# NeLy-EPFL/DeepFly3D

Measured on AMD Instinct MI355X. Metric: frames/sec (7-view 2D->3D), higher is better.
Workload: dtype f32; 1 GPU; BASELINE configs[1]: 2176 frames x 7 views 256x512x3 per GPU, 2-stack hourglass fp32, arg-max + 38-joint layout + fp64 DLT; frames_per_gpu=2176, parallelism=frame-sharded x1, one packed gather, collective_executed=False

## Files before the change

### deepfly3d_amd/csrc/hg_bt_common.h

```cpp
#pragma once
#include "hg_bt_reg.h"
#include "hg_types.h"

namespace hgk {

constexpr int BR_STAGE_BYTES = 8192;
constexpr int BR_RING = 4;
constexpr int BR_RING_BYTES = BR_RING * BR_STAGE_BYTES;
constexpr int BR_T1_PITCH = 128 * 2;
constexpr int BR_T1_BYTES = BT_HALO * BR_T1_PITCH;
__device__ __forceinline__ int br_t1_swz(int hp) { return (hp % BT_HW) & 15; }
__host__ __device__ constexpr int br_swz(int r, int c) { return (r >> 2) * 256 + (((((r & 3) << 2) | c) ^ ((r >> 3) & 3)) << 4); }
__device__ __forceinline__ void br_barrier() { asm volatile("s_waitcnt lgkmcnt(0)\n\ts_barrier" ::: "memory"); }

__device__ __forceinline__ float br_relu(float x) {
    const int b = __builtin_bit_cast(int, x);
    return __builtin_bit_cast(float, b > 0 ? b : 0);
}

template <typename I>
__device__ __forceinline__ int bt_xcd_block(I id, int n) {
    const int xcd = id & 7, q = n >> 3, r = n & 7;
    return (xcd < r ? xcd * (q + 1) : r * (q + 1) + (xcd - r) * q) + (id >> 3);
}
struct BtTile { int tx0, ty0, view; };
template <int TW, int TH, typename I>
__device__ __forceinline__ BtTile bt_tile(I id, int n, int tiles_x, int tiles_y) {
    const int b = bt_xcd_block(id, n), tx0 = (b % tiles_x) * TW, by = b / tiles_x;
    return BtTile{tx0, (by % tiles_y) * TH, by / tiles_y};
}

__device__ __forceinline__ void br_ring_issue(const void* stream, int stage, unsigned slot_addr, int wave, unsigned wvoff) {
    br_glds_stage(reinterpret_cast<const unsigned char*>(stream) + (size_t)stage * BR_STAGE_BYTES, wvoff, slot_addr + (unsigned)wave * 2048);
}

template <int HW, int HALO, int ROWB>
__device__ __forceinline__ void bt_t1_issue(const unsigned char* tin, const void* zeros, const int& tx0, const int& ty0, const int& H, const int& W, int koff,
                                            unsigned t1_addr, const int& wave, const int& lane) {
#ifdef BRF_NO_T1DMA
    return;
#endif
#pragma unroll
    for (int k = 0; k < (HALO / 4 + 3) / 4; ++k) {
        const int pc = wave + 4 * k;
        if (pc < HALO / 4) {
            const int hp = 4 * pc + (lane >> 4);
            const int hy = hp / HW, hx = hp % HW;
            const int y = ty0 - 1 + hy, x = tx0 - 1 + hx;
            const bool ok = (unsigned)y < (unsigned)H && (unsigned)x < (unsigned)W;
            const unsigned chunk = (unsigned)((lane & 15) ^ ((hp % HW) & 15));
            const unsigned char* const src = ok ? tin + ((size_t)y * W + x) * ROWB + koff + chunk * 16 : reinterpret_cast<const unsigned char*>(zeros) + chunk * 16;
            br_glds_piece64(src, t1_addr + (unsigned)pc * 1024u);
        }
    }
}
template <int HW, int HALO, int ROWB, int NH>
__device__ __forceinline__ void bt_t1_issue_persistent(const void* t1in, const void* zeros, int view, int tx0, int ty0, int H, int W, unsigned t1_addr,
                                                       int wave, unsigned uoff) {
    static_assert(NH == 1 || NH == 2, "one 64-channel half, or both");
    int lane_ = (int)(uoff >> 4);
    asm volatile("" : "+v"(lane_));
    int wave_ = wave;
    asm volatile("" : "+s"(wave_));
    const unsigned char* const tin = reinterpret_cast<const unsigned char*>(t1in) + (size_t)view * H * W * ROWB;
    const unsigned char* const zer = reinterpret_cast<const unsigned char*>(zeros);
    const int q = lane_ >> 4, slot = lane_ & 15;
    static_assert(HW >= 16, "one wrap per step of 16 halo pixels");
    const int hp0 = 4 * wave_ + q;
    int hy = hp0 / HW, hx = hp0 - hy * HW;
#pragma unroll
    for (int k = 0; k < (HALO / 4 + 3) / 4; ++k) {
        const int pc = wave_ + 4 * k;
        if (pc < HALO / 4) {
            const int y = ty0 - 1 + hy, x = tx0 - 1 + hx;
            const bool ok = (unsigned)y < (unsigned)H && (unsigned)x < (unsigned)W;
            const unsigned c16 = (unsigned)((slot ^ (hx & 15)) << 4);
            const unsigned in_view = (unsigned)((y * W + x) * ROWB) + c16;
            const unsigned char* const src = (ok ? tin : zer) + (ok ? in_view : c16);
            br_glds_piece64(src, t1_addr + (unsigned)(pc * 1024));
            if constexpr (NH == 2) br_glds_piece64(src + (ok ? 256u : 0u), t1_addr + (unsigned)(HALO * 256 + pc * 1024));
        }
        hx += 16;
        if (hx >= HW) {
            hx -= HW;
            ++hy;
        }
    }
}

template <int NT>
__device__ __forceinline__ void bt_t2_start(const float* b2, int half, f32x16 (&t2)[NT]) {
#pragma unroll
    for (int m = 0; m < NT; ++m)
#pragma unroll
        for (int q = 0; q < 4; ++q) {
            const f32x4 bb = *reinterpret_cast<const f32x4*>(b2 + 32 * m + 8 * q + 4 * half);
#pragma unroll
            for (int e = 0; e < 4; ++e) t2[m][4 * q + e] = bb[e];
        }
}
}
```

### deepfly3d_amd/csrc/hg_bt_wino_f32.h

```cpp
#pragma once
#include "hg_bt_common.h"
#include "hg_bt_reg.h"
#include "hg_bt_ring_f32.h"
#include "hg_types.h"

#ifndef WN_ABL
#define WN_ABL 0
#endif

namespace hgk {

constexpr int WN_CHUNKS = 16;
constexpr int WN_PASSES = 6;
#ifndef WN_UBUF
#define WN_UBUF 3
#endif
constexpr int WN_PASS_BYTES = 4 * 4 * 1024;
constexpr int WN_U_BYTES = 64 * WN_PASS_BYTES;
constexpr int WN_U2_BYTES = (WN_CHUNKS * WN_PASSES - 64) * WN_PASS_BYTES;
constexpr int WN_W3_BYTES = BRF_W3_STAGES * BR_STAGE_BYTES;
constexpr int WN_STREAM_BYTES = WN_U_BYTES + WN_W3_BYTES;
constexpr int WN_STREAM_BYTES_L2 = WN_U_BYTES + 2 * WN_W3_BYTES;
constexpr int WN_V_BYTES = 12 * 1024;
constexpr int WN_T1_OFF = BR_RING_BYTES;
constexpr int WN_T1_BYTES = 2 * BR_T1_BYTES;
constexpr int WN_T2_BYTES = BT_TH * BT_TW * 512;
constexpr int WN_B3_OFF = WN_T1_OFF + WN_T1_BYTES;
constexpr int WN_RING2_OFF = WN_B3_OFF + 1024 + 512;
constexpr int WN_LDS_BYTES = WN_RING2_OFF + BR_RING_BYTES;
static_assert(WN_LDS_BYTES <= 160 * 1024, "one workgroup per CU");
static_assert(WN_PASSES % WN_UBUF == 0 && WN_UBUF >= 2, "a chunk's passes use the same buffers in every chunk");
static_assert(WN_V_BYTES <= BR_RING_BYTES / 2, "V buffers 0, 1 in the W3 ring's slots 0 .. 3, buffer 2 in slots 4 .. 7");
static_assert(WN_T2_BYTES <= WN_T1_BYTES, "t2 lives in the t1 region");
static_assert(WN_U2_BYTES <= BRF_NSTAGE * BR_STAGE_BYTES, "U's second part fits the direct-form stage images");

__host__ __device__ constexpr int wn_row(int pg, int q4) { return pg >= 3 ? 3 - (q4 & 1) : (q4 & 1); }
__host__ __device__ constexpr int wn_col(int pg, int q4) { return 2 * (pg % 3) + (q4 >> 1); }

__global__ __launch_bounds__(256) void bt_wino_pack_kernel(const float* __restrict__ w2, float* __restrict__ ustream, float* __restrict__ ustream2) {
    const int idx = blockIdx.x * 256 + threadIdx.x;
    if (idx >= 128 * 128) return;
    const int co = idx >> 7, ci = idx & 127;
    double g[3][3];
#pragma unroll
    for (int ky = 0; ky < 3; ++ky)
#pragma unroll
        for (int kx = 0; kx < 3; ++kx) g[ky][kx] = (double)w2[((size_t)(ky * 3 + kx) * 128 + co) * 128 + ci];
    double t[4][3];
#pragma unroll
    for (int kx = 0; kx < 3; ++kx) {
        t[0][kx] = g[0][kx];
        t[1][kx] = 0.5 * (g[0][kx] + g[1][kx] + g[2][kx]);
        t[2][kx] = 0.5 * (g[0][kx] - g[1][kx] + g[2][kx]);
        t[3][kx] = g[2][kx];
    }
    const int c = ci >> 3, s = (ci >> 2) & 1, k = ci & 3, w = co >> 5, m = (co >> 4) & 1, r = co & 15;
#pragma unroll
    for (int pg = 0; pg < 6; ++pg)
#pragma unroll
        for (int q4 = 0; q4 < 4; ++q4) {
            const double* const x = t[wn_row(pg, q4)];
            double u;
            switch (wn_col(pg, q4)) {
                case 0: u = x[0]; break;
                case 1: u = (x[0] + x[1] + x[2]) / 3.0; break;
                case 2: u = (-x[0] + x[1] - x[2]) / 3.0; break;
                case 3: u = -(16.0 * x[0] + 8.0 * x[1] + 4.0 * x[2]) / 15.0; break;
                case 4: u = (x[0] - 2.0 * x[1] + 4.0 * x[2]) / 15.0; break;
                default: u = x[2]; break;
            }
            const int P = 6 * c + 3 * s + (pg >> 1);
            const size_t off = ((size_t)((P & 63) * 4 + w) * 4 + (pg & 1) * 2 + m) * 256 + (r + 16 * k) * 4 + q4;
            (P < 64 ? ustream : ustream2)[off] = (float)u;
        }
}
__global__ __launch_bounds__(256) void bt_wino_pack_w3_kernel(const float* __restrict__ w3, unsigned char* __restrict__ stream) {
    const int idx = blockIdx.x * 256 + threadIdx.x;
    if (idx >= BRF_W3_STAGES * 512) return;
    const int k = idx >> 9, rem = idx & 511, c = rem & 3, r = rem >> 2, nh = k >> 3, k8 = k & 7;
    const int ch = 4 * (r & 31) + (r >> 5);
    *reinterpret_cast<u32x4*>(stream + (size_t)k * BR_STAGE_BYTES + br_swz(r, c)) = *reinterpret_cast<const u32x4*>(w3 + ((size_t)nh * 128 + ch) * 128 + 16 * k8 + 4 * c);
}

__device__ __forceinline__ void wn_uload4(f32x4 (&d)[4], const void* sbase, unsigned voff) {
    asm volatile("s_nop 4\n\tglobal_load_dwordx4 %0, %4, %5\n\tglobal_load_dwordx4 %1, %4, %5 offset:1024\n\t"
                 "global_load_dwordx4 %2, %4, %5 offset:2048\n\tglobal_load_dwordx4 %3, %4, %5 offset:3072"
                 : "=&v"(d[0]), "=&v"(d[1]), "=&v"(d[2]), "=&v"(d[3])
                 : "v"(voff), "s"(sbase)
                 : "memory");
}
template <int N>
__device__ __forceinline__ void wn_uwait(f32x4 (&u)[4]) {
    asm volatile("s_waitcnt vmcnt(%4)" : "+v"(u[0]), "+v"(u[1]), "+v"(u[2]), "+v"(u[3]) : "n"(N) : "memory");
}
__device__ __forceinline__ unsigned wn_far_off(unsigned off) {
    asm volatile("" : "+s"(off));
    return off;
}
__device__ __forceinline__ void wn_xload1(f32x4& d, const void* sbase, unsigned voff) {
    asm volatile("s_nop 4\n\tglobal_load_dwordx4 %0, %1, %2" : "=&v"(d) : "v"(voff), "s"(sbase) : "memory");
}
template <int STEP>
__device__ __forceinline__ void wn_xload4s(f32x4 (&d)[4], const void* sbase, unsigned voff) {
    asm volatile("s_nop 4\n\tglobal_load_dwordx4 %0, %4, %5\n\tglobal_load_dwordx4 %1, %4, %5 offset:%6\n\t"
                 "global_load_dwordx4 %2, %4, %5 offset:%7\n\tglobal_load_dwordx4 %3, %4, %5 offset:%8"
                 : "=&v"(d[0]), "=&v"(d[1]), "=&v"(d[2]), "=&v"(d[3])
                 : "v"(voff), "s"(sbase), "n"(STEP), "n"(2 * STEP), "n"(3 * STEP)
                 : "memory");
}

template <bool UP, bool ADD2 = false, bool L2 = false>
__global__ __launch_bounds__(256, 1) void bottleneck_wino_f32_kernel(BtRingArgs p) {
    static_assert(!(UP && ADD2), "the fused up-path sum is written by plain blocks");
    static_assert(!L2 || (!UP && !ADD2), "layer2 is a plain block");
    using T = float;
    constexpr int CIN = L2 ? 128 : 256, CO = 256;
    extern __shared__ __attribute__((aligned(16))) unsigned char smem[];
    unsigned char* const ring = smem;
    unsigned char* const t1_lds = smem + WN_T1_OFF;
    float* const b3_lds = reinterpret_cast<float*>(smem + WN_B3_OFF);
    float* const b2_lds = b3_lds + 256;
    const unsigned ring_addr = lds_addr(ring), t1_addr = lds_addr(t1_lds);

    const int tid = threadIdx.x, lane = tid & 63;
    const int wave = __builtin_amdgcn_readfirstlane(tid >> 6);
    const int tiles_x = p.W / BT_TW, tiles_y = p.H / BT_TH;
    const int ntiles = p.V * tiles_y * tiles_x;
    auto tile_of = [&](int vb, int& tx0, int& ty0, int& view) {
        const BtTile t = bt_tile<BT_TW, BT_TH>(vb, ntiles, tiles_x, tiles_y);
        tx0 = t.tx0, ty0 = t.ty0, view = t.view;
    };
    unsigned uoff = (unsigned)(lane * 16);
    asm volatile("" : "+v"(uoff));
    auto t1_issue = [&](int tx0, int ty0, int view) {
        bt_t1_issue_persistent<BT_HW, BT_HALO, 512, 2>(p.t1in, p.zeros, view, tx0, ty0, p.H, p.W, t1_addr, wave, uoff);
    };


    const unsigned char* const ubase = reinterpret_cast<const unsigned char*>(p.w2d) + (size_t)wave * 4096;
    const unsigned char* const ubase2 = reinterpret_cast<const unsigned char*>(p.wstream) + (size_t)wave * 4096 - (size_t)64 * WN_PASS_BYTES;
    auto uload = [&](int c, int e, f32x4 (&dst)[4]) {
        const int P = WN_PASSES * c + e;
        wn_uload4(dst, (P < 64 ? ubase : ubase2) + (size_t)P * WN_PASS_BYTES, uoff);
    };

    const int wh = wave & 1;
    unsigned rd[6], vwr, vrd;
    auto lane_consts = [&]() {
        int l = (int)(uoff >> 4);
        asm volatile("" : "+v"(l));
        const int ppc = l & 3, pte = (l >> 2) & 3, pkq = (l >> 4) & 1, ppr = 2 * (wave >> 1) + (l >> 5);
#pragma unroll
        for (int col = 0; col < 6; ++col) {
            const int hx = 4 * ppc + col, hp = (2 * ppr + wh) * BT_HW + hx;
            rd[col] = (unsigned)(hp * 256 + ((pkq ^ (hx & 15)) << 4) + 4 * pte);
        }
        vwr = (unsigned)(((pkq * 6 + 3 * wh) * 4 + pte) * 256 + (((4 * ppr + ppc) ^ (4 * pte)) << 4));
        vrd = (unsigned)((l >> 4) * 256 + (((l & 15) ^ (4 * (l >> 4))) << 4));
    };
    auto vbuf_off = [](int b) { return b == 0 ? 0 : b == 1 ? BR_RING_BYTES / 2 : WN_RING2_OFF; };
    unsigned vrd2 = 0, vwr2 = 0;
    auto vrd_of = [&](int b) { return b == 2 ? smem + vrd2 : smem + vbuf_off(b) + vrd; };
    const f32x2 cw2 = {-1.0f, wh ? 0.0f : 1.0f}, cw0 = {0.0f, wh ? -1.0f : 0.0f};
    float tR[6][3];
    unsigned ta[6];
    auto t_addr = [&](int c) {
#pragma unroll
        for (int col = 0; col < 6; ++col) {
            ta[col] = (rd[col] ^ (unsigned)((c & 7) << 5)) + (t1_addr + (unsigned)((c >> 3) * BR_T1_BYTES));
            asm volatile("" : "+v"(ta[col]));
        }
    };
    auto t_read = [&](int col) {
        typedef const __attribute__((address_space(3))) float* lds_f;
        if (WN_ABL & 512) {
            asm volatile("" : "+v"(tR[col][0]), "+v"(tR[col][1]), "+v"(tR[col][2]));
            return;
        }
#pragma unroll
        for (int t = 0; t < 3; ++t) tR[col][t] = *(lds_f)(size_t)(ta[col] + t * BT_HW * 256);
    };
    f32x4 vo[3];
    auto t_transform = [&](int c_next_addr) {
        f32x2 x[6];
#pragma unroll
        for (int col = 0; col < 6; ++col) {
            const f32x2 P = {tR[col][0], tR[col][1]};
            if (WN_ABL & 2048) {
                x[col] = P;
                continue;
            }
            x[col] = cw0 * f32x2{tR[col][0], tR[col][0]} + (cw2 * f32x2{tR[col][2], tR[col][2]} + P);
        }
        f32x2 v[6];
        if (WN_ABL & 2048) {
#pragma unroll
            for (int j = 0; j < 6; ++j) v[j] = x[j];
        } else {
            const f32x2 h = {0.5f, 0.5f}, two = {2.0f, 2.0f};
            const f32x2 d13 = x[3] - x[1], d24 = x[4] - x[2];
            v[0] = h * d13 + (((x[0] + x[4]) - two * x[2]) + d13);
            v[1] = h * x[3] + (two * x[3] + (h * x[2] + (x[4] - x[1])));
            v[2] = h * x[3] + (((x[4] + x[1]) - two * x[2]) - h * x[2]);
            v[3] = two * (x[3] - x[1]) + d24;
            v[4] = h * (x[1] - x[3]) + d24;
            v[5] = h * d24 + (((x[5] + x[1]) - two * x[3]) + d24);
        }
#pragma unroll
        for (int jp = 0; jp < 3; ++jp) vo[jp] = f32x4{v[2 * jp][0], v[2 * jp][1], v[2 * jp + 1][0], v[2 * jp + 1][1]};
        t_addr(c_next_addr);
    };
    auto v_store = [&](int buf, int jp) {
        if (WN_ABL & 1024) {
            asm volatile("" ::"v"(vo[jp]));
            return;
        }
        *reinterpret_cast<f32x4*>((buf == 2 ? smem + vwr2 : smem + vbuf_off(buf) + vwr) + jp * 1024) = vo[jp];
    };
    auto t_transform_write = [&](int buf, int c_next_addr) {
        t_transform(c_next_addr);
#pragma unroll
        for (int jp = 0; jp < 3; ++jp) v_store(buf, jp);
    };
    auto ring_slot = [](int k) { return (k & 7) < 4 ? (k & 7) * BR_STAGE_BYTES : WN_RING2_OFF + ((k & 7) - 4) * BR_STAGE_BYTES; };
    auto ring_issue8 = [&](int set) {
        unsigned wvoff = (unsigned)wave * 2048u + uoff;
        asm volatile("" : "+v"(wvoff));
#pragma unroll
        for (int k = 8 * set; k < 8 * set + 8; ++k)
            br_ring_issue(reinterpret_cast<const unsigned char*>(p.w2d) + WN_U_BYTES, k, ring_addr + (unsigned)ring_slot(k), wave, wvoff);
    };

#ifdef DF3D_BT_TIMING
    unsigned long long stamp_ = __builtin_amdgcn_s_memtime();
#endif
    int vb = blockIdx.x;
    int tx0, ty0, view;
    tile_of(vb, tx0, ty0, view);
    t1_issue(tx0, ty0, view);
    b3_lds[tid] = L2 ? p.b3[tid] + p.bd[tid] : p.b3[tid];
    if (tid < 128) b2_lds[tid] = p.b2[tid];
    bool first = true;

#pragma unroll 1
    for (;;) {
        const int vbn = vb + (int)gridDim.x;
        const bool has_next = vbn < ntiles;
        int ntx0 = 0, nty0 = 0, nview = 0;
        if (has_next) tile_of(vbn, ntx0, nty0, nview);
        const size_t ftile = (((size_t)view * p.H + ty0 + 2 * wave) * p.W + tx0) * (CO * 4);
        const size_t htile = (((size_t)view * (p.H / 2) + ty0 / 2 + wave) * (p.W / 2) + tx0 / 2) * (CO * 4);
        const unsigned char* const xtile = reinterpret_cast<const unsigned char*>(p.in) + (L2 ? ftile / 2 : ftile);

        f32x4 acc[48];
        f32x4 ufr[WN_UBUF][4];
#pragma unroll
        for (int e = 0; e < WN_UBUF - 1; ++e) uload(0, e, ufr[e]);
        if (first) asm volatile("s_waitcnt vmcnt(%0)" ::"n"(4 * (WN_UBUF - 1)) : "memory");
        first = false;
        br_barrier();
        BR_STAMP(0);
        lane_consts();
        t_addr(0);
#pragma unroll
        for (int col = 0; col < 6; ++col) t_read(col);
        t_transform_write(0, 1);
#pragma unroll
        for (int col = 0; col < 6; ++col) t_read(col);
        t_transform_write(1, 2);
        br_barrier();
        BR_STAMP(1);

        f32x4 vf[2][2];
        auto chunk = [&](int c, auto br_tag, auto first_tag) {
            constexpr int BR = decltype(br_tag)::value;
            constexpr bool FIRST = decltype(first_tag)::value;
            const int cn = c + 1 < WN_CHUNKS ? c + 1 : c;
            const int c3 = c + 3 < WN_CHUNKS ? c + 3 : WN_CHUNKS - 1;
            const unsigned char* const vb_ = vrd_of(BR);
            if (FIRST) {
#pragma unroll
                for (int g = 0; g < 2; ++g) vf[0][g] = *reinterpret_cast<const f32x4*>(vb_ + g * 1024);
            }
#pragma unroll
            for (int e = 0; e < WN_PASSES; ++e) {
                const int pp = e % 3;
                __builtin_amdgcn_sched_barrier(0);
                if (!(WN_ABL & 1)) {
                    wn_uwait<4 * (WN_UBUF - 2)>(ufr[e % WN_UBUF]);
                    const int eu = e + WN_UBUF - 1;
                    if (eu < WN_PASSES) uload(c, eu, ufr[eu % WN_UBUF]);
                    else uload(cn, eu - WN_PASSES, ufr[eu % WN_UBUF]);
                    __builtin_amdgcn_sched_barrier(0);
                }
                if (e == 3) {
                    if (BR == 0) {
                        vwr2 = vwr + wn_far_off(WN_RING2_OFF);
                        asm volatile("" : "+v"(vwr2));
                    }
                    if (BR == 1) {
                        vrd2 = vrd + wn_far_off(WN_RING2_OFF);
                        asm volatile("" : "+v"(vrd2));
                    }
                    if (!(WN_ABL & 2)) {
                        if (WN_ABL & 4096) t_transform_write((BR + 2) % 3, c3);
                        else t_transform(c3);
                    }
                    __builtin_amdgcn_sched_barrier(0);
                }
#pragma unroll
                for (int g = 0; g < 4; ++g) {
                    if (g < 2) {
                        const int en = e + 1, sn = en / 3, ppn = en % 3;
                        if (e < WN_PASSES - 1) vf[en & 1][g] = *reinterpret_cast<const f32x4*>(vb_ + (sn * 6 + 2 * ppn + g) * 1024);
                        else vf[0][g] = *reinterpret_cast<const f32x4*>(vrd_of((BR + 1) % 3) + g * 1024);
                    }
                    if (e < 2 && g < 3 && !(WN_ABL & 2)) t_read(3 * e + g);
                    if (e == 3 && g < 3 && !(WN_ABL & (2 | 4096))) v_store((BR + 2) % 3, g);
                    const int pgl = g >> 1, m = g & 1, ai = ((2 * pp + pgl) * 2 + m) * 4;
#pragma unroll
                    for (int q4 = 0; q4 < 4; ++q4) {
                        if (FIRST && e < 3)
                            acc[ai + q4] = __builtin_amdgcn_mfma_f32_16x16x4f32(ufr[e % WN_UBUF][2 * pgl + m][q4], vf[e & 1][pgl][q4], f32x4{0.0f, 0.0f, 0.0f, 0.0f}, 0, 0, 0);
                        else
                            acc[ai + q4] = __builtin_amdgcn_mfma_f32_16x16x4f32(ufr[e % WN_UBUF][2 * pgl + m][q4], vf[e & 1][pgl][q4], acc[ai + q4], 0, 0, 0);
                    }
                    __builtin_amdgcn_sched_barrier(0);
                }
            }
            if (!(WN_ABL & 4)) br_barrier();
        };
        chunk(0, std::integral_constant<int, 0>{}, std::true_type{});
#pragma unroll 1
        for (int c = 1; c < WN_CHUNKS; c += 3) {
            chunk(c, std::integral_constant<int, 1>{}, std::false_type{});
            chunk(c + 1, std::integral_constant<int, 2>{}, std::false_type{});
            chunk(c + 2, std::integral_constant<int, 0>{}, std::false_type{});
        }
        if (!(WN_ABL & 1)) {
#pragma unroll
            for (int e = 0; e < WN_UBUF - 1; ++e) wn_uwait<0>(ufr[e]);
        }

        BR_STAMP(2);
        int lane3 = (int)(uoff >> 4);
        asm volatile("" : "+v"(lane3));
        const int half3 = lane3 >> 5, l31_3 = lane3 & 31;
        const unsigned char* const wf0 = ring + br_swz(l31_3, half3);
        const unsigned char* const wf1 = ring + br_swz(l31_3, 2 + half3);
        const int py = 2 * wave + (l31_3 >> 4), px = l31_3 & 15;
        const unsigned lane_full = (unsigned)((4 * half3 * CO + 4 * l31_3) * 4);
        const unsigned lane_half = (unsigned)((2 * half3 * CO + 4 * l31_3) * 4);
        ring_issue8(0);

        if (WN_ABL & 16) {
            float keep = 0.0f;
#pragma unroll
            for (int k = 0; k < 48; ++k) keep += acc[k][0];
            *reinterpret_cast<float*>(t1_lds + lane3 * 4) = keep;
        } else {
            const int q3 = lane3 >> 4, opr = (lane3 & 15) >> 2, opc = lane3 & 3;
#pragma unroll
            for (int m = 0; m < 2; ++m) {
                f32x4 y[2][4];
                const f32x4 bb = *reinterpret_cast<const f32x4*>(b2_lds + 32 * wave + 16 * m + 4 * q3);
#pragma unroll
                for (int reg = 0; reg < 4; ++reg) {
                    float M[4][6];
#pragma unroll
                    for (int pg = 0; pg < 6; ++pg)
#pragma unroll
                        for (int q4 = 0; q4 < 4; ++q4) M[wn_row(pg, q4)][wn_col(pg, q4)] = acc[(pg * 2 + m) * 4 + q4][reg];
                    M[1][1] += bb[reg];
                    float s[2][6];
#pragma unroll
                    for (int j = 0; j < 6; ++j) {
                        s[0][j] = M[0][j] + M[1][j] + M[2][j];
                        s[1][j] = M[1][j] - M[2][j] - M[3][j];
                    }
#pragma unroll
                    for (int a = 0; a < 2; ++a) {
                        const float sa = s[a][1] + s[a][2], sb = s[a][1] - s[a][2];
                        y[a][0][reg] = br_relu(s[a][0] + sa + s[a][3] + s[a][4]);
                        y[a][1][reg] = br_relu(sb + 0.5f * s[a][3] - 2.0f * s[a][4]);
                        y[a][2][reg] = br_relu(sa + 0.25f * s[a][3] + 4.0f * s[a][4]);
                        y[a][3][reg] = br_relu(sb + 0.125f * s[a][3] - 8.0f * s[a][4] + s[a][5]);
                    }
                }
                const int ch = 8 * wave + 4 * m + q3;
#pragma unroll
                for (int a = 0; a < 2; ++a)
#pragma unroll
                    for (int b = 0; b < 4; ++b) {
                        const int yy = 2 * opr + a, xx = 4 * opc + b;
                        *reinterpret_cast<f32x4*>(t1_lds + (yy * BT_TW + xx) * 512 + (((ch ^ (xx & 15) ^ (opr & 1)) & 31) << 4)) = y[a][b];
                    }
            }
        }
        BR_STAMP(3);
        br_wait_vm(0);
        br_barrier();
        f32x16 t2[4];
        {
            const unsigned rbase = (unsigned)((py * BT_TW + px) * 512 + ((half3 ^ (px & 15) ^ (wave & 1)) << 4));
#pragma unroll
            for (int m = 0; m < 4; ++m)
#pragma unroll
                for (int g = 0; g < 4; ++g) {
                    const f32x4 v = *reinterpret_cast<const f32x4*>(t1_lds + (rbase ^ (unsigned)((8 * m + 2 * g) << 4)));
#pragma unroll
                    for (int e = 0; e < 4; ++e) t2[m][4 * g + e] = v[e];
                }
        }

        br_barrier();
        if (has_next && !(WN_ABL & 32)) t1_issue(ntx0, nty0, nview);
        f32x4 xres[1][16];
        f32x4 exv[4];
        static_assert(!(UP && ADD2), "one extra operand");
        auto res_issue = [&](int nh) {
#pragma unroll
            for (int g = 0; g < 4; ++g) {
                if (WN_ABL & 64) {
#pragma unroll
                    for (int j = 0; j < 4; ++j) xres[0][4 * g + j] = f32x4{0.0f, 0.0f, 0.0f, 0.0f};
                } else {
                    wn_uload4(*reinterpret_cast<f32x4(*)[4]>(&xres[0][4 * g]), xtile + ((size_t)(g >> 1) * p.W + 8 * (g & 1)) * (CIN * 4) + nh * 512, lane_full);
                }
            }
            if constexpr (ADD2 || UP) {
#pragma unroll
                for (int key = 0; key < 4; ++key)
                    wn_xload1(exv[key], reinterpret_cast<const unsigned char*>(ADD2 ? p.add2 : p.in2) + htile + ((key & 1) + 4 * (key >> 1)) * (CO * 4) + nh * 512, lane_half);
            }
        };
        auto res_wait = [&](auto n_tag) {
            constexpr int N = decltype(n_tag)::value;
#pragma unroll
            for (int g = 0; g < 4; ++g) wn_uwait<N>(*reinterpret_cast<f32x4(*)[4]>(&xres[0][4 * g]));
            if constexpr (ADD2 || UP) wn_uwait<N>(exv);
        };
        if constexpr (L2) {
#pragma unroll
            for (int r = 0; r < 16; ++r)
                xres[0][r] = *reinterpret_cast<const f32x4*>(xtile + (8 * r) * 4 + (unsigned)((((l31_3 >> 4) * p.W + (l31_3 & 15)) * CIN + 4 * half3) * 4));
        } else {
            res_issue(0);
        }
        BR_STAMP(4);
#pragma unroll
        for (int nh = 0; nh < 2; ++nh) {
            f32x16 o[4];
            if (nh == 1) {
                br_wait_vm(L2 ? 16 : (ADD2 || UP) ? 36 : 32);
                br_barrier();
            }
#pragma unroll
            for (int i = 0; i < 4; ++i) {
                const float bias = b3_lds[nh * 128 + 4 * l31_3 + i];
#pragma unroll
                for (int r = 0; r < 16; ++r) o[i][r] = bias;
            }
            auto kloop = [&](auto skip_tag) {
                constexpr bool SKIP = decltype(skip_tag)::value;
#pragma unroll
                for (int k8 = 0; k8 < 8; ++k8) {
                    const int tile = k8 >> 1, q2 = k8 & 1;
#pragma unroll
                    for (int jj = 0; jj < 2; ++jj)
#pragma unroll
                        for (int i = 0; i < 4; ++i) {
                            const f32x4 wf = *reinterpret_cast<const f32x4*>((jj ? wf1 : wf0) + ring_slot(k8) + i * 2048);
                            if (WN_ABL & 256) {
                                o[i][0] += wf[0];
                                continue;
                            }
                            if constexpr (SKIP) {
                                const f32x4 xa = xres[0][2 * k8 + jj];
                                mfma_quad<T>(xa[0], xa[1], xa[2], xa[3], wf, o[i]);
                            } else {
                                mfma_quad<T>(t2[tile][8 * q2 + 4 * jj], t2[tile][8 * q2 + 4 * jj + 1], t2[tile][8 * q2 + 4 * jj + 2], t2[tile][8 * q2 + 4 * jj + 3], wf, o[i]);
                            }
                        }
                }
            };
            kloop(std::false_type{});
            if constexpr (L2) {
                br_barrier();
                ring_issue8(2 + nh);
                br_wait_vm(0);
                br_barrier();
                kloop(std::true_type{});
            }
            if (nh == 0) {
                br_barrier();
                ring_issue8(1);
            }
            BR_STAMP(5 + 2 * nh);
            if constexpr (!L2) {
                if (!(WN_ABL & 64)) {
                    if (nh == 0) res_wait(std::integral_constant<int, 16>{});
                    else res_wait(std::integral_constant<int, 0>{});
                }
            }
#pragma unroll
            for (int key = 0; key < 4; ++key) {
                const int r0 = 2 * (key & 1) + 4 * (key >> 1);
                const int hoff = ((key & 1) + 4 * (key >> 1)) * (CO * 4) + nh * 512;
                f32x4 xv[4], ov[4];
#pragma unroll
                for (int t = 0; t < 4; ++t) xv[t] = L2 ? f32x4{0.0f, 0.0f, 0.0f, 0.0f} : xres[0][r0 + (t & 1) + 8 * (t >> 1)];
                if constexpr (UP) {
#pragma unroll
                    for (int t = 0; t < 4; ++t) xv[t] += exv[key];
                }
#pragma unroll
                for (int t = 0; t < 4; ++t) {
                    const int r = r0 + (t & 1) + 8 * (t >> 1);
                    ov[t] = f32x4{o[0][r], o[1][r], o[2][r], o[3][r]};
                    if constexpr (!L2) ov[t] += xv[t];
                    if constexpr (ADD2) ov[t] += exv[key];
                    const int pl0 = (r & 3) + 8 * (r >> 2);
                    if (!(WN_ABL & 128) || ov[t][0] == 12345.678f)
                        *reinterpret_cast<f32x4*>(reinterpret_cast<unsigned char*>(p.out) + ftile + ((size_t)(pl0 >> 4) * p.W + (pl0 & 15)) * (CO * 4) + nh * 512 + lane_full) = ov[t];
                }
                auto max4 = [](const f32x4 (&v)[4]) {
                    f32x4 m;
#pragma unroll
                    for (int e = 0; e < 4; ++e) m[e] = fmaxf(fmaxf(v[0][e], v[1][e]), fmaxf(v[2][e], v[3][e]));
                    return m;
                };
                if constexpr (!UP && !L2) if (p.pool_in)
                    *reinterpret_cast<f32x4*>(reinterpret_cast<unsigned char*>(p.pool_in) + htile + hoff + lane_half) = max4(xv);
                if (p.pool) *reinterpret_cast<f32x4*>(reinterpret_cast<unsigned char*>(p.pool) + htile + hoff + lane_half) = max4(ov);
            }
            BR_STAMP(6 + 2 * nh);
            if constexpr (!L2) {
                if (nh == 0) res_issue(1);
            }
        }
        if (!has_next) break;
        vb = vbn;
        tx0 = ntx0;
        ty0 = nty0;
        view = nview;
    }
}

}
```

Before: 754.2 frames/s.

## Defer next-tile halo prefetch into the epilogue k-loop to overlap with MFMA

Moves the DMA issue of the next tile's t1 halo out of its single spot after the barrier. By default it is spread piecewise across the second-half epilogue k-loop, interleaved with the MFMA steps, and the vmcnt waits are adjusted to account for the outstanding halo loads. The aim is to stop the halo loads competing with the residual loads at the start of the epilogue and to hide their latency behind compute. In exchange the vmcnt accounting becomes more intricate, and there is a new wait before the next tile's U loads to drain the epilogue stores.

After: 756.8 frames/s, median of 6. About the same (+0.3%).

```diff
diff --git a/deepfly3d_amd/csrc/hg_bt_common.h b/deepfly3d_amd/csrc/hg_bt_common.h
--- a/deepfly3d_amd/csrc/hg_bt_common.h
+++ b/deepfly3d_amd/csrc/hg_bt_common.h
@@ -88,6 +88,27 @@
     }
 }
 
+template <int HW, int HALO, int ROWB, int NH>
+__device__ __forceinline__ void bt_t1_issue_piece(const void* t1in, const void* zeros, int view, int tx0, int ty0, int H, int W, unsigned t1_addr,
+                                                  int wave, unsigned uoff, int k) {
+    static_assert(NH == 1 || NH == 2, "one 64-channel half, or both");
+    int lane_ = (int)(uoff >> 4);
+    asm volatile("" : "+v"(lane_));
+    const int pc = wave + 4 * k;
+    if (pc >= HALO / 4) return;
+    const unsigned char* const tin = reinterpret_cast<const unsigned char*>(t1in) + (size_t)view * H * W * ROWB;
+    const unsigned char* const zer = reinterpret_cast<const unsigned char*>(zeros);
+    const int hp = 4 * pc + (lane_ >> 4), slot = lane_ & 15;
+    const int hy = hp / HW, hx = hp - hy * HW;
+    const int y = ty0 - 1 + hy, x = tx0 - 1 + hx;
+    const bool ok = (unsigned)y < (unsigned)H && (unsigned)x < (unsigned)W;
+    const unsigned c16 = (unsigned)((slot ^ (hx & 15)) << 4);
+    const unsigned in_view = (unsigned)((y * W + x) * ROWB) + c16;
+    const unsigned char* const src = (ok ? tin : zer) + (ok ? in_view : c16);
+    br_glds_piece64(src, t1_addr + (unsigned)(pc * 1024));
+    if constexpr (NH == 2) br_glds_piece64(src + (ok ? 256u : 0u), t1_addr + (unsigned)(HALO * 256 + pc * 1024));
+}
+
 template <int NT>
 __device__ __forceinline__ void bt_t2_start(const float* b2, int half, f32x16 (&t2)[NT]) {
 #pragma unroll
diff --git a/deepfly3d_amd/csrc/hg_bt_wino_f32.h b/deepfly3d_amd/csrc/hg_bt_wino_f32.h
--- a/deepfly3d_amd/csrc/hg_bt_wino_f32.h
+++ b/deepfly3d_amd/csrc/hg_bt_wino_f32.h
@@ -6,6 +6,9 @@
 
 #ifndef WN_ABL
 #define WN_ABL 0
+#endif
+#ifndef WN_HALO
+#define WN_HALO 3
 #endif
 
 namespace hgk {
@@ -30,6 +33,9 @@
 constexpr int WN_LDS_BYTES = WN_RING2_OFF + BR_RING_BYTES;
 static_assert(WN_LDS_BYTES <= 160 * 1024, "one workgroup per CU");
 static_assert(WN_PASSES % WN_UBUF == 0 && WN_UBUF >= 2, "a chunk's passes use the same buffers in every chunk");
+constexpr int WN_HALO_MIN = 2 * (BT_HALO / 4 / 4);
+constexpr int WN_EPI_STORES = (WN_ABL & 128) ? 0 : 16;
+static_assert(WN_HALO >= 0 && WN_HALO <= 3, "see WN_HALO");
 static_assert(WN_V_BYTES <= BR_RING_BYTES / 2, "V buffers 0, 1 in the W3 ring's slots 0 .. 3, buffer 2 in slots 4 .. 7");
 static_assert(WN_T2_BYTES <= WN_T1_BYTES, "t2 lives in the t1 region");
 static_assert(WN_U2_BYTES <= BRF_NSTAGE * BR_STAGE_BYTES, "U's second part fits the direct-form stage images");
@@ -254,6 +260,7 @@
 
         f32x4 acc[48];
         f32x4 ufr[WN_UBUF][4];
+        if (WN_HALO >= 2 && !first) br_wait_vm(WN_EPI_STORES);
 #pragma unroll
         for (int e = 0; e < WN_UBUF - 1; ++e) uload(0, e, ufr[e]);
         if (first) asm volatile("s_waitcnt vmcnt(%0)" ::"n"(4 * (WN_UBUF - 1)) : "memory");
@@ -287,7 +294,7 @@
                 const int pp = e % 3;
                 __builtin_amdgcn_sched_barrier(0);
                 if (!(WN_ABL & 1)) {
-                    wn_uwait<4 * (WN_UBUF - 2)>(ufr[e % WN_UBUF]);
+                    wn_uwait<(WN_ABL & 8192) ? 63 : 4 * (WN_UBUF - 2)>(ufr[e % WN_UBUF]);
                     const int eu = e + WN_UBUF - 1;
                     if (eu < WN_PASSES) uload(c, eu, ufr[eu % WN_UBUF]);
                     else uload(cn, eu - WN_PASSES, ufr[eu % WN_UBUF]);
@@ -414,7 +421,14 @@
         }
 
         br_barrier();
-        if (has_next && !(WN_ABL & 32)) t1_issue(ntx0, nty0, nview);
+        auto halo_issue = [&]() {
+            if (has_next && !(WN_ABL & 32)) t1_issue(ntx0, nty0, nview);
+        };
+        auto halo_piece = [&](int k) {
+            if (has_next && !(WN_ABL & 32))
+                bt_t1_issue_piece<BT_HW, BT_HALO, 512, 2>(p.t1in, p.zeros, nview, ntx0, nty0, p.H, p.W, t1_addr, wave, uoff, k);
+        };
+        if (WN_HALO == 0) halo_issue();
         f32x4 xres[1][16];
         f32x4 exv[4];
         static_assert(!(UP && ADD2), "one extra operand");
@@ -435,7 +449,7 @@
             }
         };
         auto res_wait = [&](auto n_tag) {
-            constexpr int N = decltype(n_tag)::value;
+            constexpr int N = (WN_ABL & 16384) ? 63 : decltype(n_tag)::value;
 #pragma unroll
             for (int g = 0; g < 4; ++g) wn_uwait<N>(*reinterpret_cast<f32x4(*)[4]>(&xres[0][4 * g]));
             if constexpr (ADD2 || UP) wn_uwait<N>(exv);
@@ -447,6 +461,7 @@
         } else {
             res_issue(0);
         }
+        if (WN_HALO == 1) halo_issue();
         BR_STAMP(4);
 #pragma unroll
         for (int nh = 0; nh < 2; ++nh) {
@@ -454,6 +469,7 @@
             if (nh == 1) {
                 br_wait_vm(L2 ? 16 : (ADD2 || UP) ? 36 : 32);
                 br_barrier();
+                if (WN_HALO == 2 && !L2) halo_issue();
             }
 #pragma unroll
             for (int i = 0; i < 4; ++i) {
@@ -461,13 +477,15 @@
 #pragma unroll
                 for (int r = 0; r < 16; ++r) o[i][r] = bias;
             }
-            auto kloop = [&](auto skip_tag) {
+            auto kloop = [&](auto skip_tag, auto halo_tag) {
                 constexpr bool SKIP = decltype(skip_tag)::value;
+                constexpr bool HSTEPS = decltype(halo_tag)::value;
 #pragma unroll
                 for (int k8 = 0; k8 < 8; ++k8) {
                     const int tile = k8 >> 1, q2 = k8 & 1;
 #pragma unroll
-                    for (int jj = 0; jj < 2; ++jj)
+                    for (int jj = 0; jj < 2; ++jj) {
+                        if (HSTEPS && 2 * k8 + jj < 12) halo_piece(2 * k8 + jj);
 #pragma unroll
                         for (int i = 0; i < 4; ++i) {
                             const f32x4 wf = *reinterpret_cast<const f32x4*>((jj ? wf1 : wf0) + ring_slot(k8) + i * 2048);
@@ -482,15 +500,18 @@
                                 mfma_quad<T>(t2[tile][8 * q2 + 4 * jj], t2[tile][8 * q2 + 4 * jj + 1], t2[tile][8 * q2 + 4 * jj + 2], t2[tile][8 * q2 + 4 * jj + 3], wf, o[i]);
                             }
                         }
+                    }
                 }
             };
-            kloop(std::false_type{});
+            if (WN_HALO == 3 && !L2 && nh == 1) kloop(std::false_type{}, std::true_type{});
+            else kloop(std::false_type{}, std::false_type{});
             if constexpr (L2) {
                 br_barrier();
                 ring_issue8(2 + nh);
                 br_wait_vm(0);
                 br_barrier();
-                kloop(std::true_type{});
+                if (WN_HALO >= 2 && nh == 1) halo_issue();
+                kloop(std::true_type{}, std::false_type{});
             }
             if (nh == 0) {
                 br_barrier();
@@ -499,8 +520,14 @@
             BR_STAMP(5 + 2 * nh);
             if constexpr (!L2) {
                 if (!(WN_ABL & 64)) {
-                    if (nh == 0) res_wait(std::integral_constant<int, 16>{});
-                    else res_wait(std::integral_constant<int, 0>{});
+                    constexpr int H0 = WN_HALO == 1 && !(WN_ABL & 32) ? WN_HALO_MIN : 0, H1 = WN_HALO >= 2 && !(WN_ABL & 32) ? WN_HALO_MIN : 0;
+                    if (nh == 0) {
+                        if (H0 && !has_next) br_wait_vm((WN_ABL & 16384) ? 63 : 16);
+                        res_wait(std::integral_constant<int, 16 + H0>{});
+                    } else {
+                        if (H1 && !has_next) br_wait_vm((WN_ABL & 16384) ? 63 : 0);
+                        res_wait(std::integral_constant<int, H1>{});
+                    }
                 }
             }
 #pragma unroll
```
